# QWTforGithub/CDSegNet

Hardware: AMD Instinct MI355X
Metric: points/sec/node (ScanNet ~120k-pt scenes, 1-step) (higher is better)
Workload: dtype f16

## Files before the change

### cdsegnet_amd/_lib.py

```python
import ctypes
import os
import threading
from ctypes import POINTER, Structure, c_char_p, c_float, c_int, c_int32, c_int64, c_long, c_size_t, c_uint64, c_void_p

HERE = os.path.dirname(os.path.abspath(__file__))
LIB_PATH = os.path.join(HERE, "libcdseg_hip.so")
LIB_PATH_F16 = os.path.join(HERE, "libcdseg_hip_f16.so")

F32, BF16 = 0, 1
ACT_NONE, ACT_GELU, ACT_SWISH = 0, 1, 2
ORDER_IDS = {"z": 0, "z-trans": 1, "hilbert": 2, "hilbert-trans": 3}
ERRORS = {-1: "CDSEG_ERR_ARG", -2: "CDSEG_ERR_LAUNCH", -3: "CDSEG_ERR_WORKSPACE", -4: "CDSEG_ERR_UNSUPPORTED"}


class CdsegError(RuntimeError):
    pass


class DuplicateVoxelsError(CdsegError):

    def __init__(self, msg, count):
        super().__init__(msg)
        self.count = int(count)

# ... 143 lines not shown
    "cdseg_attn_tail_rr": (c_int, [c_void_p, c_int, c_void_p, c_void_p, c_void_p, c_void_p, c_float, c_void_p, c_void_p,
                                   c_void_p, c_int, c_void_p, c_int, c_long, c_int, c_void_p]),
    "cdseg_cpe_head_rr2": (c_int, [c_void_p, c_int, c_void_p, c_void_p, c_void_p, c_void_p, c_void_p, c_int, c_void_p, c_int,
                                   c_void_p, c_void_p, c_void_p, c_float, c_void_p, c_void_p, c_int, c_long, c_int, c_int, c_void_p]),
    "cdseg_attn_tail_rr2": (c_int, [c_void_p, c_int, c_void_p, c_void_p, c_void_p, c_void_p, c_float, c_void_p, c_void_p,
                                    c_void_p, c_int, c_void_p, c_int, c_void_p, c_int, c_long, c_int, c_void_p, c_size_t, c_void_p]),
    "cdseg_block_scratch_bytes": (c_size_t, [POINTER(BlockDesc), c_long]),
    "cdseg_block_forward": (c_int, [POINTER(BlockDesc), POINTER(BlockIO), c_void_p]),
    "cdseg_layernorm": (c_int, [c_void_p, c_int, c_int, c_void_p, c_void_p, c_float, c_void_p, c_int, c_void_p,
                                c_void_p, c_int, c_int, c_void_p, c_int, c_int, c_long, c_int, c_void_p]),
    "cdseg_attention": (c_int, [c_void_p, c_void_p, c_void_p, c_int, c_int, c_int, c_void_p, c_void_p, c_void_p,
                                c_void_p, c_int, c_int, c_int, c_float, c_void_p, c_int, c_int, c_void_p]),
    "cdseg_attention_ex": (c_int, [c_void_p, c_void_p, c_void_p, c_int, c_int, c_int, c_void_p, c_void_p, c_void_p,
                                   c_void_p, c_int, c_int, c_int, c_float, c_void_p, c_int, c_int, c_int, c_void_p]),
    "cdseg_attention_schedule": (c_long, [c_int, c_int, c_int, c_int, c_void_p, c_long]),
    "cdseg_attention_bwd_ws_bytes": (c_size_t, [c_long, c_int]),
    "cdseg_attention_bwd": (c_int, [c_void_p, c_void_p, c_void_p, c_int, c_int, c_int, c_void_p, c_void_p, c_void_p, c_void_p,
                                    c_int, c_int, c_long, c_int, c_float, c_void_p, c_int, c_void_p, c_void_p, c_void_p,
                                    c_int, c_int, c_int, c_int, c_void_p, c_size_t, c_void_p]),
    "cdseg_layernorm_bwd": (c_int, [c_void_p, c_int, c_void_p, c_float, c_void_p, c_int, c_void_p, c_int, c_int, c_void_p,
                                    c_void_p, c_long, c_int, c_void_p]),
    "cdseg_gelu_bwd": (c_int, [c_void_p, c_void_p, c_void_p, c_long, c_void_p]),
    "cdseg_conv_wgrad": (c_int, [c_void_p, c_int, c_void_p, c_int, c_void_p, c_int, c_long, c_int, c_int, c_void_p, c_void_p,
                                 c_void_p]),
    "cdseg_linear_wgrad": (c_int, [c_void_p, c_int, c_void_p, c_void_p, c_int, c_long, c_int, c_int, c_void_p, c_int, c_void_p,
                                   c_void_p]),
    "cdseg_prof_enable": (c_int, [c_int]),
    "cdseg_prof_summary": (c_int, [POINTER(ctypes.c_double), POINTER(c_long)]),
    "cdseg_prof_summary_class": (c_int, [c_int, POINTER(ctypes.c_double), POINTER(c_long)]),
    "cdseg_segment_max": (c_int, [c_void_p, c_int, c_int, c_void_p, c_long, c_int, c_void_p, c_void_p, c_int,
# ... 74 lines not shown
```

### cdsegnet_amd/csrc/gemm.hip

```cpp
#include <cstdlib>

#include <atomic>

#include "common.h"
#include "prof.h"

#ifndef CDSEG_CONV_SQ128_MIN_M
#define CDSEG_CONV_SQ128_MIN_M 8000
#endif
#ifndef CDSEG_CONV_SQ128_MAX_M
#define CDSEG_CONV_SQ128_MAX_M 32768
#endif

namespace {

struct GemmP {
  const void* A;
  const void* W;
  const float* bias;
  const float* scale;
  const float* shift;
  const float* res;
  const float* add_src;
  const int32_t* add_idx;
// ... 1 lines not shown
  const int32_t* out_idx;
  void* out;
  void* out2;
  long M;
  int N, K, kvol;
  int lda, ldo, ldo2, ldres, ldadd;
  int out_dtype, out2_dtype;
  int act, out2_pre_add;
  int vec_ok;
  float* ws;
  int splits;
  int kshift;
  long nbr_sm, nbr_so;
  int gm, gn;
  int xmode;
  int fix;
  const float* colbias;
  const float* ln_pre_g;
  const float* ln_pre_b;
  const float* ln_post_g;
  const float* ln_post_b;
  void* ln_out;
  int ldln, ln_out_dtype;
  float ln_eps;
  int alt;
#ifdef CDSEG_EXPERIMENTS
  int dbg;
#endif
};

// ... 252 lines not shown
  const long groups = g.M * (long)(g.N >> 2);
  const long t = (long)blockIdx.x * blockDim.x + threadIdx.x;
  if (t >= groups) return;
  const long m = t / (g.N >> 2);
  const int n = (int)(t - m * (g.N >> 2)) << 2;
  const long stride = g.M * (long)g.N;
  const float* p = g.ws + m * g.N + n;
  float4 v = *reinterpret_cast<const float4*>(p);
  for (int s = 1; s < g.splits; ++s) {
    const float4 u = *reinterpret_cast<const float4*>(p + s * stride);
    v.x += u.x; v.y += u.y; v.z += u.z; v.w += u.w;
  }
  epilogue4(g, m, n, v);
}

__global__ __launch_bounds__(256) void row_finish_kernel(GemmP g) {
  const int lane = threadIdx.x & 63;
  const long m = (long)blockIdx.x * 4 + (threadIdx.x >> 6);
  if (m >= g.M) return;
  const int groups = g.N >> 2;
  const long sstride = g.M * (long)g.N;
  float4 v[2];
#pragma unroll
  for (int i = 0; i < 2; ++i) {
    v[i] = make_float4(0.f, 0.f, 0.f, 0.f);
    if (lane + 64 * i < groups) {
      const float* p = g.ws + m * g.N + 4 * (lane + 64 * i);
      v[i] = *reinterpret_cast<const float4*>(p);
      for (int s2 = 1; s2 < g.splits; ++s2) {
        const float4 u = *reinterpret_cast<const float4*>(p + s2 * sstride);
// ... 8 lines not shown
__device__ unsigned long long g_gemm_t[8 * 16384];
extern "C" int cdseg_debug_gemm_timing(unsigned long long* host_dst, size_t count) {
  return hipMemcpyFromSymbol(host_dst, HIP_SYMBOL(g_gemm_t), count * sizeof(unsigned long long)) == hipSuccess ? 0 : -2;
}
__device__ unsigned long long g_gemm_kt[4096 * 16 * 8];
extern "C" int cdseg_debug_gemm_ktiming(unsigned long long* host_dst, size_t count) {
  return hipMemcpyFromSymbol(host_dst, HIP_SYMBOL(g_gemm_kt), count * sizeof(unsigned long long)) == hipSuccess ? 0 : -2;
}
#define KT_STAMP(x) const unsigned long long x = __builtin_readcyclecounter()
#else
#define KT_STAMP(x)
#endif

template <int BN, int BM, bool SQ = false, int AI = 2, int AJ = BN / 32>
__device__ __forceinline__ void tile_epilogue(const GemmP& g, f32x4_t (&acc)[AI][AJ], char* smem, int tid, int lane,
                                              int wm, int wn, long m0, int n0, int zs) {
  constexpr int NT = SQ ? 512 : 4 * BM;
  constexpr int TN = BN / 32;
  constexpr int CLD = BN + 4;
  const int fr = lane & 15, fg = lane >> 4;
  float* Cs = reinterpret_cast<float*>(smem);
  const bool plain = !g.fix && plain_bf16_out(g);
  Cols8 cols;
  if (plain) cols = load_cols8(g, n0 + 8 * (tid % (BN / 8)));
  auto lds_barrier = [] {
    asm volatile("s_waitcnt lgkmcnt(0)" ::: "memory");
    __builtin_amdgcn_s_barrier();
  };
#pragma unroll 1
  for (int hh = 0; hh < BM / 64; ++hh) {
#ifdef CDSEG_GEMM_TIMING
    if (tid == 0 && blockIdx.x < 16384) g_gemm_t[(size_t)blockIdx.x * 8 + 4 + 2 * hh] = __builtin_readcyclecounter();
#endif
    if (hh) lds_barrier();
    int zcol = 0;
    if constexpr (BM > 64) asm volatile("v_mov_b32 %0, 0" : "=v"(zcol));
    if constexpr (SQ) {
// ... 9 lines not shown
      const int rbase = (wm & 1) * 32;
#pragma unroll
      for (int i = 0; i < 2; ++i)
#pragma unroll
        for (int j = 0; j < TN; ++j)
#pragma unroll
          for (int r = 0; r < 4; ++r)
            Cs[(rbase + i * 16 + fg * 4 + r) * CLD + wn * (BN / 2) + j * 16 + fr] = acc[i][j][r];
    }
    lds_barrier();
#ifdef CDSEG_GEMM_TIMING
    if (tid == 0 && blockIdx.x < 16384) g_gemm_t[(size_t)blockIdx.x * 8 + 5 + 2 * hh] = __builtin_readcyclecounter();
#endif
    const long mb = m0 + 64 * hh;
    constexpr int GPR = BN / 4;
    if (g.fix) {
      for (int item = tid; item < 64 * GPR; item += NT) {
        const int row = item / GPR, cg = item % GPR;
        const long m = mb + row;
        const int n = n0 + 4 * cg;
        if (m >= g.M || n >= g.N) continue;
        *reinterpret_cast<float4*>(g.ws + ((long)zs * g.M + m) * g.N + n) =
            *reinterpret_cast<const float4*>(Cs + row * CLD + 4 * cg);
      }
    } else if (BM == 64 && (g.ln_pre_g || g.ln_post_g)) {
      constexpr int MAXG = BN / 16;
      const int row = (tid >> 2) & 63, part = tid & 3;
      const long m = mb + row;
      const int ng = g.N >> 2;
      float4 v[MAXG];
#pragma unroll
      for (int i = 0; i < MAXG; ++i)
        v[i] = (part + 4 * i < ng) ? *reinterpret_cast<const float4*>(Cs + row * CLD + 4 * (part + 4 * i))
                                   : make_float4(0.f, 0.f, 0.f, 0.f);
      finish_row<MAXG>(g, m, m < g.M, part, 4, ng, 0, v);
    } else if (plain) {
      static_assert(NT % (GPR / 2) == 0, "a lane's columns must not change between items");
// ... 254 lines not shown
              for (int j = 0; j < TN; ++j)
                acc[i][j] = __builtin_amdgcn_mfma_f32_16x16x4f32(a[i][h][ss], b[j][h][ss], acc[i][j], 0, 0, 0);
      }
    }
    __syncthreads();
    if (kc + 1 < kc1) store_tiles();
    __syncthreads();
  }

  if constexpr (kIsX3<CT>) {
#pragma unroll
    for (int i = 0; i < 2; ++i)
#pragma unroll
      for (int j = 0; j < TN; ++j) acc[i][j] += accx[i][j] * (1.0f / 2048.f);
  }
  tile_epilogue<BN, BM>(g, acc, smem, tid, lane, wm, wn, m0, n0, zs);
}

__device__ uint4 g_zero_page[8];

template <int BM, bool GATHER = true, int BN = 128, int NST = 2, bool SQ = false>
struct DmaCfg {
  static constexpr int WAVES = SQ ? 8 : BM / 16, NT = WAVES * 64, BK = 64;
  static constexpr int A_BYTES = BM * 128, W_BYTES = BN * 128;
  static constexpr int A_PW = (BM / 8) / WAVES, W_PW = (BN / 8) / WAVES;
  static constexpr int STAGES = NST * (A_BYTES + W_BYTES);
  static constexpr int ITAB = GATHER ? BM * 27 * 4 : 0;
  static constexpr int LDS = STAGES + ITAB + 1024;
};

template <int BM, bool GATHER, int BN = 128, int NST = 2, bool SQ = false>
// ... 5 lines not shown
  constexpr int TN = BN / 32;
  constexpr int AI = SQ ? 4 : 2, AJ = TN;
  static_assert(!SQ || (BM == 256 && NST == 2 && GATHER), "SQ: 256-row tiles of 8 waves, two stages, sparse convs");
  extern __shared__ __attribute__((aligned(16))) char smem[];
  char* tail = smem + D::STAGES + D::ITAB;
  int* live = reinterpret_cast<int*>(tail);
  int* glive = reinterpret_cast<int*>(tail + 256);
  unsigned long long* smask = reinterpret_cast<unsigned long long*>(tail + 640);
  int* itab = reinterpret_cast<int*>(smem + D::STAGES);

  const int tid = threadIdx.x;
  const int lane = tid & 63;
  const int wave = __builtin_amdgcn_readfirstlane(tid >> 6);
  const int wm = wave >> 1, wn = wave & 1;
  int mt, sl;
  {
    const int bid = blockIdx.x, slices = g.gn * g.splits;
    if (g.xmode == 1) {
      const int j = bid >> 3;
      mt = j % g.gm;
      sl = (bid & 7) + 8 * (j / g.gm);
      if (sl >= slices) return;
    } else if (g.xmode == 2) {
      const int j = bid >> 3, chunk = (g.gm + 7) >> 3;
      mt = (bid & 7) * chunk + j / slices;
      sl = j % slices;
      if (j / slices >= chunk || mt >= g.gm) return;
    } else {
      mt = bid % g.gm;
      sl = bid / g.gm;
    }
  }
  const int nt = sl % g.gn, zs = sl / g.gn;
// ... 37 lines not shown
    __syncthreads();
    nlive = __builtin_amdgcn_readfirstlane(live[0]);
#pragma unroll
    for (int i = 0; i < PASSES; ++i) {
      const int o = og + OPT * i;
      if (o < g.kvol) {
        const int sl2 = slotmap[o];
        if (sl2 >= 0) itab[r * 27 + sl2] = idx[i];
      }
    }
    __syncthreads();
  }
  const int KV = nlive * g.K;
  const int nkc = KV / D::BK;
  const int kshift = g.kshift;
  const int kc0 = (int)(((long)nkc * zs) / g.splits);
  const int kc1 = (int)(((long)nkc * (zs + 1)) / g.splits);

  const int lrow = lane >> 3, slot = lane & 7;
  const bf16_t* a_src[D::A_PW];
  int a_row[D::A_PW];
  int a_chunk[D::A_PW];
  const bf16_t* w_src[D::W_PW];
  int w_chunk[D::W_PW];
#pragma unroll
  for (int i = 0; i < D::A_PW; ++i) {
    const int r = (wave * D::A_PW + i) * 8 + lrow;
    a_row[i] = r;
    a_chunk[i] = slot ^ ((r >> 1) & 7);
    long m = m0 + r;
    if (m >= g.M) m = g.M - 1;
    a_src[i] = (const bf16_t*)g.A + m * g.lda + a_chunk[i] * 8;
// ... 217 lines not shown
  }
#ifdef CDSEG_GEMM_TIMING
  if (lane == 0 && blockIdx.x < 4096 && wave < 16) {
    unsigned long long* d = g_gemm_kt + ((size_t)blockIdx.x * 16 + wave) * 8;
    d[0] = kt_wait; d[1] = kt_bar; d[2] = kt_issue; d[3] = kt_mma; d[4] = (unsigned long long)(kc1 - kc0); d[5] = kt_pro;
    d[6] = (unsigned long long)nlive; d[7] = 1;
  }
#endif
  __syncthreads();
#ifdef CDSEG_EXPERIMENTS
  if (g.dbg & 4) { if (acc[0][0][0] == 12345.678f) ((float*)g.out)[0] = acc[1][1][1]; return; }
#endif
#ifdef CDSEG_GEMM_TIMING
  const unsigned long long tc1 = __builtin_readcyclecounter();
#endif
  tile_epilogue<BN, BM, SQ, AI, AJ>(g, acc, smem, tid, lane, wm, wn, m0, n0, zs);
#ifdef CDSEG_GEMM_TIMING
  if (tid == 0 && blockIdx.x < 16384) {
    unsigned long long* d = g_gemm_t + (size_t)blockIdx.x * 8;
    d[0] = rt0; d[1] = __builtin_amdgcn_s_memrealtime(); d[2] = tc1 - tc0;
    const unsigned long long tend = __builtin_readcyclecounter();
    d[3] = tend - tc1;
    const unsigned long long a0 = d[4], a1 = d[5], b0 = d[6], b1 = d[7];
    d[4] = a1 - a0; d[5] = b0 - a1; d[6] = b1 - b0; d[7] = tend - b1;
  }
#endif
}

thread_local bool tl_leave_partials = false;
thread_local int tl_partial_splits = 1;

template <typename CT, int BN, int NCH, int BM>
constexpr int gemm_smem_bytes() {
  constexpr int ab = (BM + BN) * NCH * 16, c = 64 * (BN + 4) * 4;
  return (ab > c ? ab : c) + 1024;
}


template <typename CT, int NCH, bool GATHER>
int launch_bn(GemmP p, size_t ws_bytes, hipStream_t s) {
  constexpr int BK = NCH * (16 / (int)sizeof(CT));
  static const int split_target = cdseg_knob("CDSEG_GEMM_SPLIT_TARGET", 320);
  static const int split_max = cdseg_knob("CDSEG_GEMM_SPLIT_MAX", 16);
  static const int xmode_env = cdseg_knob("CDSEG_GEMM_XMODE", -1);
  const bool ln = p.ln_pre_g || p.ln_post_g;
// ... 71 lines not shown
  else if (ln && gn > 1) p.fix = 2;
  if (p.fix) {
    if (!can_fix || (size_t)splits * p.M * p.N * sizeof(float) > ws_bytes) return CDSEG_ERR_WORKSPACE;
    if (p.fix == 2 && p.N > 512) return CDSEG_ERR_UNSUPPORTED;
  }
  p.splits = splits;
  p.gm = gm;
  p.gn = gn;
  const int slices = gn * splits;
  const long wbytes = (long)p.N * p.kvol * p.K * (long)sizeof(CT);
  p.xmode = 0;
  if (sq) p.xmode = gm >= 64 ? 2 : 0;
  else if (slices >= 8 && wbytes >= (1 << 20) && gm > 1) p.xmode = 1;
  else if (GATHER && gm >= 64) p.xmode = 2;
  if (xmode_env >= 0) p.xmode = (xmode_env == 1 && slices < 8) ? 0 : xmode_env;
  unsigned nblk;
  if (p.xmode == 1) nblk = 8u * (unsigned)((slices + 7) / 8) * (unsigned)gm;
  else if (p.xmode == 2) nblk = 8u * (unsigned)((gm + 7) / 8) * (unsigned)slices;
  else nblk = (unsigned)gm * (unsigned)slices;
  const dim3 grid(nblk);
  bool launched = false;
  if constexpr (NCH == 16 && sizeof(CT) == 2) {
    static const int dma_on = cdseg_knob("CDSEG_GEMM_DMA", 1);
    static const int dma_bm = cdseg_knob("CDSEG_GEMM_DMA_BM", 0);
    const bool fused_ln_here = ln && gn == 1 && splits == 1;
    if constexpr (GATHER) {
      if (sq && dma_on && sq_bn == 128) {
        launched = true;
        using Q = DmaCfg<256, true, 128, 2, true>;
        static std::atomic<bool> aq128{false};
        if (!aq128) {
          if (hipFuncSetAttribute((const void*)gemm_dma_kernel<256, true, 128, 2, true>, hipFuncAttributeMaxDynamicSharedMemorySize,
// ... 117 lines not shown
            attr_x3 = true;
          }
          hipLaunchKernelGGL((gemm_kernel<CT, 128, NCH, false, 128>), grid, dim3(512), smem, s, p);
        } else {
          hipLaunchKernelGGL((gemm_kernel<CT, 128, NCH, false, 128>), grid, dim3(512), 0, s, p);
        }
      }
    }
  }
  if (!launched) {
    if (bn == 32) hipLaunchKernelGGL((gemm_kernel<CT, 32, NCH, GATHER>), grid, dim3(256), 0, s, p);
    else if (bn == 64) hipLaunchKernelGGL((gemm_kernel<CT, 64, NCH, GATHER>), grid, dim3(256), 0, s, p);
    else hipLaunchKernelGGL((gemm_kernel<CT, 128, NCH, GATHER>), grid, dim3(256), 0, s, p);
  }
  if (hipGetLastError() != hipSuccess) return CDSEG_ERR_LAUNCH;
  if (p.fix == 2) {
    hipLaunchKernelGGL(row_finish_kernel, dim3((unsigned)((p.M + 3) / 4)), dim3(256), 0, s, p);
    if (hipGetLastError() != hipSuccess) return CDSEG_ERR_LAUNCH;
  } else if (p.fix == 1) {
    if (tl_leave_partials && p.vec_ok && p.bias && !p.scale && p.act == CDSEG_ACT_NONE && !p.res && !p.add_src && !p.out2 &&
        !p.out_idx && !p.colbias) {
      tl_partial_splits = p.splits;
      return CDSEG_OK;
    }
    const long groups = p.M * (long)(p.N >> 2);
    hipLaunchKernelGGL(splitk_epilogue_kernel, dim3((unsigned)((groups + 255) / 256)), dim3(256), 0, s, p);
    if (hipGetLastError() != hipSuccess) return CDSEG_ERR_LAUNCH;
  }
  return CDSEG_OK;
}
// ... 39 lines not shown
  p.colbias = a->colbias; p.ln_pre_g = a->ln_pre_g; p.ln_pre_b = a->ln_pre_b; p.ln_post_g = a->ln_post_g;
  p.ln_post_b = a->ln_post_b; p.ln_out = a->ln_out; p.ldln = a->ldln; p.ln_out_dtype = a->ln_out_dtype;
  p.ln_eps = a->ln_eps;
  if (p.ln_pre_g || p.ln_post_g) {
    if (a->N > 512 || !p.vec_ok || a->out_idx || (p.ln_pre_g && !p.ln_pre_b) || (p.ln_post_g && (!p.ln_post_b || !a->ln_out)) ||
        (a->ln_out && (a->ldln % 4)))
      return CDSEG_ERR_UNSUPPORTED;
  }
  if (p.colbias && !al16(p.colbias)) p.vec_ok = 0;
  p.ws = (a->ws && ((((uintptr_t)a->ws) & 15) == 0)) ? (float*)a->ws : nullptr;
  p.splits = 1;
  p.fix = 0;
  p.alt = cdseg_knob("CDSEG_GEMM_ALT", 0);
  p.gm = p.gn = 1;
  p.xmode = 0;
  p.kshift = -1;
  if ((a->K & (a->K - 1)) == 0) {
    int sh = 0;
    while ((1 << sh) < a->K) ++sh;
    p.kshift = sh;
  }
  const size_t wsb = p.ws ? a->ws_bytes : 0;
  hipStream_t s = (hipStream_t)stream;
  CdsegProfToken tok;
  const bool prof = a->nbr && a->kvol == 27 && cdseg_prof_begin(CDSEG_PROF_CONV_DEEP, s, &tok);
  int rc = CDSEG_ERR_ARG;
  if (a->compute_dtype == CDSEG_BF16) rc = a->nbr ? launch<bf16_t, true>(p, wsb, s) : launch<bf16_t, false>(p, wsb, s);
  else if (a->compute_dtype == CDSEG_F32) rc = a->nbr ? launch<float, true>(p, wsb, s) : launch<float, false>(p, wsb, s);
  else if (a->compute_dtype == CDSEG_F32X3) rc = a->nbr ? launch<F32X3, true>(p, wsb, s) : launch<F32X3, false>(p, wsb, s);
  if (prof) cdseg_prof_end(tok, s);
  return rc;
}

int gemm_leave_partials(const cdseg_gemm_args* a, int* splits, void* stream) {
  tl_leave_partials = true;
  tl_partial_splits = 1;
  const int rc = cdseg_gemm(a, stream);
  tl_leave_partials = false;
  *splits = tl_partial_splits;
  return rc;
}
```

### cdsegnet_amd/csrc/runtime.hip

```cpp
#include <cstdlib>
#include <cstring>

#include "common.h"
#include "deep.h"

namespace {

inline size_t align_up(size_t v, size_t a) { return (v + a - 1) / a * a; }

struct Carver {
  char* base;
  size_t off, cap;
  void* take(size_t bytes) {
    off = align_up(off, 256);
    void* p = base ? base + off : nullptr;
    off += bytes;
    return p;
  }
};

constexpr int FUSE_LN_MAX_C = 512;
constexpr size_t SPLITK_WS_CAP = (size_t)64 << 20;

inline size_t esz(int dtype) { return dtype == CDSEG_BF16 ? 2 : 4; }
// ... 11 lines not shown
  Layout L;
  L.y = c.take(n * C * e);
  L.h = c.take(n * C * e);
  L.qkv = c.take(n * 3 * C * e);
  L.o = c.take(n * C * e);
  L.u = c.take(n * (size_t)d->hidden * e);
  L.y2 = d->channels > FUSE_LN_MAX_C ? c.take(n * C * 4) : nullptr;
  const long tiles = ((n + 63) / 64) * (((long)C + 127) / 128);
  L.ws_bytes = tiles < 256 ? (size_t)32 * n * (size_t)(3 * C > (size_t)d->hidden ? 3 * C : d->hidden) * 4
                           : (C > 128 ? (size_t)n * C * 4 : 0);
  if (C >= 256 && ((n + 127) / 128) * (((long)C + 255) / 256) < 256) {
    const size_t want = (size_t)8 * n * C * 4;
    if (want > L.ws_bytes) L.ws_bytes = want;
  }
  if (L.ws_bytes > SPLITK_WS_CAP) L.ws_bytes = SPLITK_WS_CAP;
  L.ws = L.ws_bytes ? c.take(L.ws_bytes) : nullptr;
  L.xs = (d->dtype == CDSEG_BF16 && C >= 128 && d->head_img && d->tail_img) ? c.take(n * C * 4) : nullptr;
  L.total = align_up(c.off, 256);
  return L;
}

cdseg_gemm_args base_args(const cdseg_block_desc* d, const Layout& L, long n) {
  cdseg_gemm_args a;
  std::memset(&a, 0, sizeof(a));
  a.M = n;
  a.kvol = 1;
  a.a_dtype = storage_dtype(d->dtype);
  a.compute_dtype = d->dtype;
  a.ws = L.ws;
  a.ws_bytes = L.ws_bytes;
// ... 192 lines not shown
```

### cdsegnet_amd/ops.py

```python
import ctypes
import os
import threading

import torch

from . import _lib
from ._lib import ACT_GELU, ACT_NONE, ACT_SWISH, BF16, F32, GemmArgs, check

__all__ = ["ACT_NONE", "ACT_GELU", "ACT_SWISH", "F32", "BF16"]

LP_DTYPES = {"bf16": torch.bfloat16, "f16": torch.float16}


class _Dtypes:

    def __getitem__(self, dtype):
        if dtype == torch.float32:
            return F32
        if dtype == LP_DTYPES[_lib.active()]:
            return BF16
        raise _lib.CdsegError(f"{dtype} tensors do not belong to the active build of the library ({_lib.active()})")


_DT = _Dtypes()
# ... 441 lines not shown
        patch = (ctypes.c_int * k)(*[int(it[3]) for it in chunk])
        npad = (ctypes.c_long * k)(*[int(it[4]) for it in chunk])
        check(lib.cdseg_pad_plan_batch(k, orders, offs, offs_pad, patch, npad, int(nb), _ptr(gidx), _ptr(widx), _stream()),
              "pad_plan_batch")
        sizes = [int(it[4]) for it in chunk]
        res.extend(zip(gidx.split(sizes), widx.split(sizes)))
    return res


F32X3 = 2


def set_f32x3(on):
    prev, _TLS.f32x3 = _TLS.f32x3, bool(on)
    return prev


def gemm(A, W, out, *, bias=None, scale=None, shift=None, act=ACT_NONE, res=None, add_src=None, add_idx=None,
         nbr=None, out_idx=None, out2=None, out2_pre_add=False, M=None, kvol=1, colbias=None, ln_pre=None,
         nbr_kmajor=False,
         ln_post=None, ln_out=None, ln_eps=1e-5, cache=True):
    if not A.is_cuda:
        _need_gpu(A, W, out)
    x3 = _TLS.f32x3 and W.dtype == torch.float32
    key = (W.data_ptr(), _dp(bias), _dp(scale), _dp(shift), int(kvol), int(act), x3)
    cache_d = _TLS.gemm_cache
    ent = cache_d.get(key) if cache else None
    if ent is None:
        for t in (bias, scale, shift):
            if t is not None and t.dtype != torch.float32:
# ... 27 lines not shown
    a.a_dtype = _DT[A.dtype]
    a.out_dtype = _DT[out.dtype]
    a.out2_dtype = _DT[out2.dtype] if out2 is not None else 0
    a.out2_pre_add = 1 if out2_pre_add else 0
    a.colbias = _dp(colbias)
    if ln_pre is not None:
        a.ln_pre_g, a.ln_pre_b = ln_pre[0].data_ptr(), ln_pre[1].data_ptr()
    else:
        a.ln_pre_g = a.ln_pre_b = None
    if ln_post is not None:
        a.ln_post_g, a.ln_post_b = ln_post[0].data_ptr(), ln_post[1].data_ptr()
        a.ln_out, a.ldln, a.ln_out_dtype = ln_out.data_ptr(), ln_out.stride(0), _DT[ln_out.dtype]
    else:
        a.ln_post_g = a.ln_post_b = a.ln_out = None
    a.ln_eps = float(ln_eps)
    if ((m + 63) >> 6) * ((a.N + 127) >> 7) < 256:
        ws = workspace(min(32 * m * a.N * 4, 64 << 20), out.device)
        a.ws, a.ws_bytes = ws.data_ptr(), ws.numel()
    elif nbr is not None and a.N >= 256 and ((m + 127) >> 7) * ((a.N + 255) >> 8) < 256:
        ws = workspace(min(8 * m * a.N * 4, 64 << 20), out.device)
        a.ws, a.ws_bytes = ws.data_ptr(), ws.numel()
    elif a.N > 128 and (ln_pre is not None or ln_post is not None):
        ws = workspace(m * a.N * 4, out.device)
        a.ws, a.ws_bytes = ws.data_ptr(), ws.numel()
    else:
        a.ws, a.ws_bytes = None, 0
    tok = TIMER.begin("conv" if nbr is not None else "gemm") if TIMER is not None else None
    check(_lib.load().cdseg_gemm(ent[1], _stream()), "gemm")
    if tok is not None:
        TIMER.end(tok, 2.0 * a.M * a.N * a.K * a.kvol)
    return out


FUSED_MLP_CHANNELS = (32, 64, 128)

# ... 534 lines not shown
```

### include/cdseg.h

```cpp
#ifndef CDSEG_H
#define CDSEG_H

#include <stddef.h>
#include <stdint.h>

#ifdef __cplusplus
extern "C" {
#endif

#define CDSEG_OK 0
#define CDSEG_ERR_ARG (-1)
#define CDSEG_ERR_LAUNCH (-2)
#define CDSEG_ERR_WORKSPACE (-3)
#define CDSEG_ERR_UNSUPPORTED (-4)

#define CDSEG_F32 0
#define CDSEG_BF16 1
#define CDSEG_F32X3 2

#define CDSEG_ORDER_Z 0
#define CDSEG_ORDER_Z_TRANS 1
#define CDSEG_ORDER_HILBERT 2
#define CDSEG_ORDER_HILBERT_TRANS 3

// ... 98 lines not shown
int cdseg_layernorm(const void* x, int x_dtype, int ldx, const float* gamma, const float* beta, float eps,
                    const float* res, int ldres, const float* colbias, void* out, int out_dtype, int ldo,
                    void* out2, int out2_dtype, int ldo2, long m, int c, void* stream);

int cdseg_attention(const void* q, const void* k, const void* v, int ldq, int ldk, int ldv, const int32_t* q_gidx,
                    const int32_t* kv_gidx, const int32_t* widx, const int32_t* patch_start, int num_patches,
                    int num_heads, int max_len, float scale, void* out, int ldo, int dtype, void* stream);
#define CDSEG_ATTN_Q_PRESCALED 1
#define CDSEG_ATTN_V_BF16 2
int cdseg_attention_ex(const void* q, const void* k, const void* v, int ldq, int ldk, int ldv, const int32_t* q_gidx,
                       const int32_t* kv_gidx, const int32_t* widx, const int32_t* patch_start, int num_patches,
                       int num_heads, int max_len, float scale, void* out, int ldo, int dtype, int flags, void* stream);

long cdseg_attention_schedule(int num_patches, int num_heads, int max_len, int dtype, int32_t* table, long capacity);

int cdseg_prof_enable(int on);
int cdseg_prof_summary(double* total_ms, long* launches);
#define CDSEG_PROF_ATTENTION 0
#define CDSEG_PROF_CONV 1
#define CDSEG_PROF_CONV_DEEP 2
int cdseg_prof_summary_class(int cls, double* total_ms, long* launches);

int cdseg_segment_max(const void* y, int y_dtype, int ldy, const int32_t* seg_start, long m, int c,
                      const float* scale, const float* shift, int act, float* out, int ldo, void* out2,
                      int out2_dtype, int ldo2, void* stream);
size_t cdseg_pool_fused_img_bytes(int cin, int cout);
int cdseg_pool_fused_pack(const void* w, int cin, int cout, void* wimg, void* stream);
int cdseg_pool_fused(const void* x, int ldx, const void* wimg, const float* bias, const int32_t* seg_start, long m,
                     const float* scale, const float* shift, int act, float* out, int ldo, void* out2, int ldo2,
                     int cin, int cout, void* stream);
// ... 213 lines not shown
```

Baseline: 79.83 million.

## Add cost-model split plan for sparse conv GEMM with per-tile mixed split-K

Adds a host-side planner that picks, per XCD, how many output tiles run whole and how many are split across K into S or S+1 pieces, replacing uniform split-K for 256x256 gathered bf16 convolutions. The goal is to balance the tail of the wave across compute slots and cut partial-sum traffic compared with splitting every tile. Partial tiles are written to a compact workspace and reduced by a new epilogue kernel. This adds planning cost (cached), extra workspace sizing in Python and the runtime, and depends on hand-tuned cost constants.

```diff
diff --git a/cdsegnet_amd/_lib.py b/cdsegnet_amd/_lib.py
--- a/cdsegnet_amd/_lib.py
+++ b/cdsegnet_amd/_lib.py
@@ -181,6 +181,8 @@
     "cdseg_attention_ex": (c_int, [c_void_p, c_void_p, c_void_p, c_int, c_int, c_int, c_void_p, c_void_p, c_void_p,
                                    c_void_p, c_int, c_int, c_int, c_float, c_void_p, c_int, c_int, c_int, c_void_p]),
     "cdseg_attention_schedule": (c_long, [c_int, c_int, c_int, c_int, c_void_p, c_long]),
+    "cdseg_conv_split_plan_ws_bytes": (c_size_t, [c_long, c_int, c_int]),
+    "cdseg_debug_conv_split_plan": (c_long, [c_long, c_int, c_int, c_size_t, c_void_p, POINTER(c_size_t), c_void_p, c_long]),
     "cdseg_attention_bwd_ws_bytes": (c_size_t, [c_long, c_int]),
     "cdseg_attention_bwd": (c_int, [c_void_p, c_void_p, c_void_p, c_int, c_int, c_int, c_void_p, c_void_p, c_void_p, c_void_p,
                                     c_int, c_int, c_long, c_int, c_float, c_void_p, c_int, c_void_p, c_void_p, c_void_p,
diff --git a/cdsegnet_amd/csrc/gemm.hip b/cdsegnet_amd/csrc/gemm.hip
--- a/cdsegnet_amd/csrc/gemm.hip
+++ b/cdsegnet_amd/csrc/gemm.hip
@@ -1,6 +1,9 @@
 #include <cstdlib>
 
+#include <algorithm>
 #include <atomic>
+#include <mutex>
+#include <vector>
 
 #include "common.h"
 #include "prof.h"
@@ -39,6 +42,7 @@
   long nbr_sm, nbr_so;
   int gm, gn;
   int xmode;
+  int pw, pnb, ps;
   int fix;
   const float* colbias;
   const float* ln_pre_g;
@@ -321,6 +325,72 @@
   epilogue4(g, m, n, v);
 }
 
+struct PlanXcd {
+  int row0, w, nb, nc;
+  int chi;
+};
+__host__ __device__ __forceinline__ PlanXcd plan_xcd(int gm, int gn, int pw, int pnb, int x) {
+  const int base = gm >> 3, rem = gm & 7;
+  const int T = (base + (x < rem ? 1 : 0)) * gn, thi = (base + (rem ? 1 : 0)) * gn;
+  const int whi = pw < thi ? pw : thi;
+  PlanXcd o;
+  o.row0 = x * base + (x < rem ? x : rem);
+  o.w = pw < T ? pw : T;
+  o.nb = pnb < T - o.w ? pnb : T - o.w;
+  o.nc = T - o.w - o.nb;
+  o.chi = thi - whi - (pnb < thi - whi ? pnb : thi - whi);
+  return o;
+}
+struct PlanPiece {
+  int mt, nt, a, S;
+  int wt;
+};
+__host__ __device__ __forceinline__ bool plan_decode(int gm, int gn, int pw, int pnb, int ps, int bid, PlanPiece& o) {
+  const int x = bid & 7, j = bid >> 3;
+  const PlanXcd c = plan_xcd(gm, gn, pw, pnb, x);
+  int t;
+  if (j < c.w) {
+    t = j; o.a = 0; o.S = 1; o.wt = -1;
+  } else if (j < c.w + c.nb * ps) {
+    const int jj = j - c.w, a = jj / c.nb, k = jj - a * c.nb;
+    t = c.w + k; o.a = a; o.S = ps; o.wt = (a * 8 + x) * pnb + k;
+  } else {
+    const int jj = j - c.w - c.nb * ps;
+    if (jj >= c.nc * (ps + 1)) return false;
+    const int a = jj / c.nc, k = jj - a * c.nc;
+    t = c.w + c.nb + k; o.a = a; o.S = ps + 1; o.wt = 8 * pnb * ps + (a * 8 + x) * c.chi + k;
+  }
+  o.mt = c.row0 + t / gn;
+  o.nt = t - (t / gn) * gn;
+  return true;
+}
+
+template <int BM, int BN>
+__global__ __launch_bounds__(256) void plan_epilogue_kernel(GemmP g) {
+  const PlanXcd c0 = plan_xcd(g.gm, g.gn, g.pw, g.pnb, 0);
+  const int per = g.pnb + c0.chi;
+  const int x = blockIdx.y / per, k = blockIdx.y - x * per;
+  const PlanXcd c = plan_xcd(g.gm, g.gn, g.pw, g.pnb, x);
+  const bool late = k >= g.pnb;
+  const int kk = late ? k - g.pnb : k;
+  if (kk >= (late ? c.nc : c.nb)) return;
+  const int t = c.w + (late ? c.nb : 0) + kk, S = g.ps + (late ? 1 : 0);
+  const long slot0 = late ? (long)8 * g.pnb * g.ps + x * c.chi + kk : (long)x * g.pnb + kk;
+  const long sstride = (long)8 * (late ? c.chi : g.pnb) * (BM * BN);
+  const int item = blockIdx.x * 256 + threadIdx.x;
+  const int row = item / (BN / 4), cg = item - row * (BN / 4);
+  const long m = (long)(c.row0 + t / g.gn) * BM + row;
+  const int n = (t % g.gn) * BN + 4 * cg;
+  if (m >= g.M || n >= g.N) return;
+  const float* p = g.ws + slot0 * (BM * BN) + row * BN + 4 * cg;
+  float4 v = *reinterpret_cast<const float4*>(p);
+  for (int s = 1; s < S; ++s) {
+    const float4 u = *reinterpret_cast<const float4*>(p + s * sstride);
+    v.x += u.x; v.y += u.y; v.z += u.z; v.w += u.w;
+  }
+  epilogue4(g, m, n, v);
+}
+
 __global__ __launch_bounds__(256) void row_finish_kernel(GemmP g) {
   const int lane = threadIdx.x & 63;
   const long m = (long)blockIdx.x * 4 + (threadIdx.x >> 6);
@@ -359,13 +429,13 @@
 
 template <int BN, int BM, bool SQ = false, int AI = 2, int AJ = BN / 32>
 __device__ __forceinline__ void tile_epilogue(const GemmP& g, f32x4_t (&acc)[AI][AJ], char* smem, int tid, int lane,
-                                              int wm, int wn, long m0, int n0, int zs) {
+                                              int wm, int wn, long m0, int n0, int fix, float* wsp, long wld) {
   constexpr int NT = SQ ? 512 : 4 * BM;
   constexpr int TN = BN / 32;
   constexpr int CLD = BN + 4;
   const int fr = lane & 15, fg = lane >> 4;
   float* Cs = reinterpret_cast<float*>(smem);
-  const bool plain = !g.fix && plain_bf16_out(g);
+  const bool plain = !fix && plain_bf16_out(g);
   Cols8 cols;
   if (plain) cols = load_cols8(g, n0 + 8 * (tid % (BN / 8)));
   auto lds_barrier = [] {
@@ -405,13 +475,13 @@
 #endif
     const long mb = m0 + 64 * hh;
     constexpr int GPR = BN / 4;
-    if (g.fix) {
+    if (fix) {
       for (int item = tid; item < 64 * GPR; item += NT) {
         const int row = item / GPR, cg = item % GPR;
         const long m = mb + row;
         const int n = n0 + 4 * cg;
         if (m >= g.M || n >= g.N) continue;
-        *reinterpret_cast<float4*>(g.ws + ((long)zs * g.M + m) * g.N + n) =
+        *reinterpret_cast<float4*>(wsp + (long)(64 * hh + row) * wld + 4 * cg) =
             *reinterpret_cast<const float4*>(Cs + row * CLD + 4 * cg);
       }
     } else if (BM == 64 && (g.ln_pre_g || g.ln_post_g)) {
@@ -696,7 +766,7 @@
 #pragma unroll
       for (int j = 0; j < TN; ++j) acc[i][j] += accx[i][j] * (1.0f / 2048.f);
   }
-  tile_epilogue<BN, BM>(g, acc, smem, tid, lane, wm, wn, m0, n0, zs);
+  tile_epilogue<BN, BM>(g, acc, smem, tid, lane, wm, wn, m0, n0, g.fix, g.ws + ((long)zs * g.M + m0) * g.N + n0, g.N);
 }
 
 __device__ uint4 g_zero_page[8];
@@ -732,9 +802,14 @@
   const int wave = __builtin_amdgcn_readfirstlane(tid >> 6);
   const int wm = wave >> 1, wn = wave & 1;
   int mt, sl;
+  int pS = 0, pz = 0, pwt = -1;
   {
     const int bid = blockIdx.x, slices = g.gn * g.splits;
-    if (g.xmode == 1) {
+    if (SQ && g.xmode == 3) {
+      PlanPiece pp;
+      if (!plan_decode(g.gm, g.gn, g.pw, g.pnb, g.ps, bid, pp)) return;
+      mt = pp.mt; sl = pp.nt; pS = pp.S; pz = pp.a; pwt = pp.wt;
+    } else if (g.xmode == 1) {
       const int j = bid >> 3;
       mt = j % g.gm;
       sl = (bid & 7) + 8 * (j / g.gm);
@@ -802,8 +877,13 @@
   const int KV = nlive * g.K;
   const int nkc = KV / D::BK;
   const int kshift = g.kshift;
-  const int kc0 = (int)(((long)nkc * zs) / g.splits);
-  const int kc1 = (int)(((long)nkc * (zs + 1)) / g.splits);
+  int kc0 = (int)(((long)nkc * zs) / g.splits);
+  int kc1 = (int)(((long)nkc * (zs + 1)) / g.splits);
+  if (SQ && pS) {
+    const int q = nkc / pS, r = nkc - q * pS;
+    kc0 = pz * q + (pz < r ? pz : r);
+    kc1 = kc0 + q + (pz < r ? 1 : 0);
+  }
 
   const int lrow = lane >> 3, slot = lane & 7;
   const bf16_t* a_src[D::A_PW];
@@ -1051,7 +1131,12 @@
 #ifdef CDSEG_GEMM_TIMING
   const unsigned long long tc1 = __builtin_readcyclecounter();
 #endif
-  tile_epilogue<BN, BM, SQ, AI, AJ>(g, acc, smem, tid, lane, wm, wn, m0, n0, zs);
+  {
+    const bool planned = SQ && pS;
+    const int fix = planned ? (pwt >= 0 ? 1 : 0) : g.fix;
+    float* wsp = planned ? g.ws + (long)pwt * (BM * BN) : g.ws + ((long)zs * g.M + m0) * g.N + n0;
+    tile_epilogue<BN, BM, SQ, AI, AJ>(g, acc, smem, tid, lane, wm, wn, m0, n0, fix, wsp, planned ? (long)BN : (long)g.N);
+  }
 #ifdef CDSEG_GEMM_TIMING
   if (tid == 0 && blockIdx.x < 16384) {
     unsigned long long* d = g_gemm_t + (size_t)blockIdx.x * 8;
@@ -1066,6 +1151,136 @@
 
 thread_local bool tl_leave_partials = false;
 thread_local int tl_partial_splits = 1;
+
+constexpr double PLAN_STEP_US = 1.65;
+constexpr double PLAN_PARTIAL_US = 0.11;
+constexpr double PLAN_PASS_US = 2.0;
+constexpr int PLAN_PIECE_STEPS = 3;
+constexpr int PLAN_SLOTS = 32;
+constexpr int PLAN_MAX_S = 7;
+constexpr double PLAN_MIN_GAIN = 0.03;
+constexpr size_t PLAN_TILE_BYTES = (size_t)256 * 256 * 4;
+
+struct SplitPlan {
+  int uniform;
+  int pw, pnb, ps;
+  int nblk;
+  int makespan;
+  int partials;
+  long ws_tiles;
+  double cost_us;
+};
+
+int plan_makespan(int T, int pw, int pnb, int ps, int nkc) {
+  const int w = pw < T ? pw : T, nb = pnb < T - w ? pnb : T - w, nc = T - w - nb;
+  int slot[PLAN_SLOTS] = {0};
+  int end = 0;
+  auto put = [&](int len) {
+    int b = 0;
+    for (int i = 1; i < PLAN_SLOTS; ++i)
+      if (slot[i] < slot[b]) b = i;
+    slot[b] += len + PLAN_PIECE_STEPS;
+    if (slot[b] > end) end = slot[b];
+  };
+  for (int i = 0; i < w; ++i) put(nkc);
+  for (int cls = 0; cls < 2; ++cls) {
+    const int S = ps + cls, cnt = cls ? nc : nb;
+    if (!cnt) continue;
+    const int q = nkc / S, r = nkc - q * S;
+    for (int a = 0; a < S; ++a)
+      for (int k = 0; k < cnt; ++k) put(q + (a < r ? 1 : 0));
+  }
+  return end;
+}
+
+SplitPlan conv_split_plan(int gm, int gn, int nkc, size_t ws_bytes, int usplits, bool leave) {
+  struct Key { int gm, gn, nkc, us, leave; size_t cap; };
+  struct Ent { Key k; SplitPlan p; };
+  static std::mutex mu;
+  static std::vector<Ent> cache;
+  const Key key{gm, gn, nkc, usplits, leave ? 1 : 0, ws_bytes / PLAN_TILE_BYTES};
+  {
+    std::lock_guard<std::mutex> lk(mu);
+    for (const Ent& e : cache)
+      if (e.k.gm == key.gm && e.k.gn == key.gn && e.k.nkc == key.nkc && e.k.us == key.us && e.k.leave == key.leave &&
+          e.k.cap == key.cap)
+        return e.p;
+  }
+  const int base = gm >> 3, rem = gm & 7;
+  const int thi = (base + (rem ? 1 : 0)) * gn, tlo = base * gn;
+  SplitPlan best;
+  best.uniform = 1; best.pw = best.pnb = best.ps = 0; best.nblk = 0; best.partials = 0; best.ws_tiles = 0;
+  {
+    const long per = gm >= 64 ? (long)((gm + 7) / 8) * gn * usplits : ((long)gm * gn * usplits + 7) / 8;
+    const int len = (nkc + usplits - 1) / usplits + PLAN_PIECE_STEPS;
+    best.makespan = (int)((per + PLAN_SLOTS - 1) / PLAN_SLOTS) * len;
+    best.cost_us = best.makespan * PLAN_STEP_US;
+    if (usplits > 1) best.cost_us += (double)gm * gn * usplits * PLAN_PARTIAL_US + (leave ? 0.0 : PLAN_PASS_US);
+  }
+  const double need = best.cost_us * (1.0 - PLAN_MIN_GAIN);
+  SplitPlan plan = best;
+  plan.cost_us = 1e30;
+  struct Cand { double floor_us, fixed; int pw, pnb, ps, parts; long tiles; };
+  std::vector<Cand> cands;
+  for (int pw = thi > 48 ? thi - 48 : 0; pw <= thi; ++pw) {
+    const int R = thi - pw;
+    for (int ps = 2; ps <= PLAN_MAX_S; ++ps) {
+      if (nkc / (ps + 1) < 8) break;
+      if (R == 0 && ps > 2) break;
+      for (int pnb = (R && ps > 2) ? 1 : 0; pnb <= R; ++pnb) {
+        const PlanXcd c = plan_xcd(gm, gn, pw, pnb, 0);
+        const long tiles = (long)8 * pnb * ps + (long)8 * c.chi * (ps + 1);
+        if ((size_t)tiles > ws_bytes / PLAN_TILE_BYTES) continue;
+        int parts = 0;
+        for (int x = 0; x < 8; ++x) {
+          const PlanXcd cx = plan_xcd(gm, gn, pw, pnb, x);
+          parts += cx.nb * ps + cx.nc * (ps + 1);
+        }
+        const long work = (long)c.w * (nkc + PLAN_PIECE_STEPS) + (long)c.nb * (nkc + ps * PLAN_PIECE_STEPS) +
+                          (long)c.nc * (nkc + (ps + 1) * PLAN_PIECE_STEPS);
+        const double fixed = parts * PLAN_PARTIAL_US + (parts ? PLAN_PASS_US : 0.0);
+        const double floor_us = (double)((work + PLAN_SLOTS - 1) / PLAN_SLOTS) * PLAN_STEP_US + fixed;
+        if (floor_us < need) cands.push_back(Cand{floor_us, fixed, pw, pnb, ps, parts, tiles});
+      }
+    }
+  }
+  std::sort(cands.begin(), cands.end(), [](const Cand& a, const Cand& b) {
+    if (a.floor_us != b.floor_us) return a.floor_us < b.floor_us;
+    if (a.parts != b.parts) return a.parts < b.parts;
+    return a.pw != b.pw ? a.pw < b.pw : (a.ps != b.ps ? a.ps < b.ps : a.pnb < b.pnb);
+  });
+  for (const Cand& cd : cands) {
+    if (cd.floor_us >= plan.cost_us) break;
+    int ms = plan_makespan(thi, cd.pw, cd.pnb, cd.ps, nkc);
+    if (tlo != thi && tlo > 0) {
+      const int m2 = plan_makespan(tlo, cd.pw, cd.pnb, cd.ps, nkc);
+      if (m2 > ms) ms = m2;
+    }
+    const double cost = ms * PLAN_STEP_US + cd.fixed;
+    if (cost < plan.cost_us) {
+      const PlanXcd c = plan_xcd(gm, gn, cd.pw, cd.pnb, 0);
+      plan.uniform = 0; plan.pw = cd.pw; plan.pnb = cd.pnb; plan.ps = cd.ps; plan.makespan = ms; plan.partials = cd.parts;
+      plan.ws_tiles = cd.tiles; plan.cost_us = cost;
+      plan.nblk = 8 * (c.w + c.nb * cd.ps + c.nc * (cd.ps + 1));
+    }
+  }
+  if (plan.cost_us < need) best = plan;
+  std::lock_guard<std::mutex> lk(mu);
+  if (cache.size() > 256) cache.clear();
+  cache.push_back(Ent{key, best});
+  return best;
+}
+
+int sq_uniform_splits(long M, int N, int K, int gm, int gn, size_t ws_bytes) {
+  const long nkc128 = ((long)27 * K + 127) / 128, blocks = (long)gm * gn;
+  if (blocks >= 256 || nkc128 < 4) return 1;
+  int smax = (int)(nkc128 / 2);
+  if (smax > 16) smax = 16;
+  while (smax > 1 && (size_t)smax * M * N * sizeof(float) > ws_bytes) --smax;
+  int splits = (int)(256 / blocks);
+  if (splits > smax) splits = smax;
+  return splits < 1 ? 1 : splits;
+}
 
 template <typename CT, int BN, int NCH, int BM>
 constexpr int gemm_smem_bytes() {
@@ -1167,8 +1382,37 @@
   else if (slices >= 8 && wbytes >= (1 << 20) && gm > 1) p.xmode = 1;
   else if (GATHER && gm >= 64) p.xmode = 2;
   if (xmode_env >= 0) p.xmode = (xmode_env == 1 && slices < 8) ? 0 : xmode_env;
+  SplitPlan plan;
+  plan.uniform = 1;
+  if constexpr (GATHER && NCH == 16 && sizeof(CT) == 2) {
+    static const int plan_on = cdseg_knob("CDSEG_CONV_SPLIT_PLAN", 1);
+    if (plan_on && sq && sq_bn == 256 && can_fix && xmode_env < 0 && p.fix != 2) {
+      const bool leave = tl_leave_partials && p.bias && !p.scale && p.act == CDSEG_ACT_NONE && !p.res && !p.add_src && !p.out2 &&
+                         !p.colbias;
+      plan = conv_split_plan(gm, gn, (int)((long)p.kvol * p.K / 64), ws_bytes, splits, leave);
+#ifdef CDSEG_EXPERIMENTS
+      if (const int fps = cdseg_knob("CDSEG_PLAN_PS", 0); fps > 0) {
+        const int fpw = cdseg_knob("CDSEG_PLAN_PW", 0), fpnb = cdseg_knob("CDSEG_PLAN_PNB", 0);
+        const PlanXcd c = plan_xcd(gm, gn, fpw, fpnb, 0);
+        const long tiles = (long)8 * fpnb * fps + (long)8 * c.chi * (fps + 1);
+        if ((size_t)tiles <= ws_bytes / PLAN_TILE_BYTES) {
+          plan.uniform = 0; plan.pw = fpw; plan.pnb = fpnb; plan.ps = fps; plan.ws_tiles = tiles;
+          plan.partials = c.nb + c.nc;
+          plan.nblk = 8 * (c.w + c.nb * fps + c.nc * (fps + 1));
+        }
+      }
+#endif
+      if (!plan.uniform) {
+        p.splits = 1;
+        p.fix = 0;
+        p.xmode = 3;
+        p.pw = plan.pw; p.pnb = plan.pnb; p.ps = plan.ps;
+      }
+    }
+  }
   unsigned nblk;
-  if (p.xmode == 1) nblk = 8u * (unsigned)((slices + 7) / 8) * (unsigned)gm;
+  if (p.xmode == 3) nblk = (unsigned)plan.nblk;
+  else if (p.xmode == 1) nblk = 8u * (unsigned)((slices + 7) / 8) * (unsigned)gm;
   else if (p.xmode == 2) nblk = 8u * (unsigned)((gm + 7) / 8) * (unsigned)slices;
   else nblk = (unsigned)gm * (unsigned)slices;
   const dim3 grid(nblk);
@@ -1316,6 +1560,14 @@
     else hipLaunchKernelGGL((gemm_kernel<CT, 128, NCH, GATHER>), grid, dim3(256), 0, s, p);
   }
   if (hipGetLastError() != hipSuccess) return CDSEG_ERR_LAUNCH;
+  if (p.xmode == 3) {
+    if (plan.partials) {
+      const unsigned per = (unsigned)(p.pnb + plan_xcd(gm, gn, p.pw, p.pnb, 0).chi);
+      hipLaunchKernelGGL((plan_epilogue_kernel<256, 256>), dim3(256 * 256 / 1024, 8u * per), dim3(256), 0, s, p);
+      if (hipGetLastError() != hipSuccess) return CDSEG_ERR_LAUNCH;
+    }
+    return CDSEG_OK;
+  }
   if (p.fix == 2) {
     hipLaunchKernelGGL(row_finish_kernel, dim3((unsigned)((p.M + 3) / 4)), dim3(256), 0, s, p);
     if (hipGetLastError() != hipSuccess) return CDSEG_ERR_LAUNCH;
@@ -1385,6 +1637,7 @@
   p.alt = cdseg_knob("CDSEG_GEMM_ALT", 0);
   p.gm = p.gn = 1;
   p.xmode = 0;
+  p.pw = p.pnb = p.ps = 0;
   p.kshift = -1;
   if ((a->K & (a->K - 1)) == 0) {
     int sh = 0;
@@ -1411,3 +1664,37 @@
   *splits = tl_partial_splits;
   return rc;
 }
+
+extern "C" size_t cdseg_conv_split_plan_ws_bytes(long M, int N, int K) {
+  if (M < 5000 || N < 256 || (N % 256) || K <= 0 || (K & (K - 1)) || K < 64) return 0;
+  const int gm = (int)((M + 255) / 256), gn = N / 256;
+  const size_t big = ~(size_t)0 >> 1;
+  const SplitPlan pl = conv_split_plan(gm, gn, 27 * K / 64, big, sq_uniform_splits(M, N, K, gm, gn, big), false);
+  return pl.uniform ? 0 : (size_t)pl.ws_tiles * PLAN_TILE_BYTES;
+}
+
+extern "C" long cdseg_debug_conv_split_plan(long M, int N, int K, size_t ws_bytes, int32_t* hdr, size_t* ws_need, int32_t* pieces,
+                                            long capacity) {
+  if (!hdr || !ws_need || M < 5000 || N < 256 || (N % 256) || K <= 0 || (K & (K - 1)) || K < 64) return CDSEG_ERR_ARG;
+  const int gm = (int)((M + 255) / 256), gn = N / 256, nkc = 27 * K / 64;
+  const int us = sq_uniform_splits(M, N, K, gm, gn, ws_bytes);
+  const SplitPlan pl = conv_split_plan(gm, gn, nkc, ws_bytes, us, false);
+  const int h[12] = {pl.uniform, us, gm, gn, nkc, pl.pw, pl.pnb, pl.ps, pl.nblk, pl.makespan, pl.partials, 0};
+  for (int i = 0; i < 12; ++i) hdr[i] = h[i];
+  *ws_need = pl.uniform ? (us > 1 ? (size_t)us * M * N * sizeof(float) : 0) : (size_t)pl.ws_tiles * PLAN_TILE_BYTES;
+  if (pl.uniform) return 0;
+  for (long b = 0; b < pl.nblk && b < capacity && pieces; ++b) {
+    int32_t* o = pieces + 6 * b;
+    PlanPiece pp;
+    if (!plan_decode(gm, gn, pl.pw, pl.pnb, pl.ps, (int)b, pp)) {
+      for (int i = 0; i < 6; ++i) o[i] = -1;
+      continue;
+    }
+    const int q = nkc / pp.S, r = nkc - q * pp.S;
+    o[0] = (int)(b & 7); o[1] = pp.mt; o[2] = pp.nt;
+    o[3] = pp.a * q + (pp.a < r ? pp.a : r);
+    o[4] = o[3] + q + (pp.a < r ? 1 : 0);
+    o[5] = pp.wt;
+  }
+  return pl.nblk;
+}
diff --git a/cdsegnet_amd/csrc/runtime.hip b/cdsegnet_amd/csrc/runtime.hip
--- a/cdsegnet_amd/csrc/runtime.hip
+++ b/cdsegnet_amd/csrc/runtime.hip
@@ -49,6 +49,10 @@
     if (want > L.ws_bytes) L.ws_bytes = want;
   }
   if (L.ws_bytes > SPLITK_WS_CAP) L.ws_bytes = SPLITK_WS_CAP;
+  if (C >= 256 && d->dtype == CDSEG_BF16) {
+    const size_t want = cdseg_conv_split_plan_ws_bytes(n, (int)C, (int)C);
+    if (want > L.ws_bytes) L.ws_bytes = want;
+  }
   L.ws = L.ws_bytes ? c.take(L.ws_bytes) : nullptr;
   L.xs = (d->dtype == CDSEG_BF16 && C >= 128 && d->head_img && d->tail_img) ? c.take(n * C * 4) : nullptr;
   L.total = align_up(c.off, 256);
diff --git a/cdsegnet_amd/ops.py b/cdsegnet_amd/ops.py
--- a/cdsegnet_amd/ops.py
+++ b/cdsegnet_amd/ops.py
@@ -479,6 +479,19 @@
 def set_f32x3(on):
     prev, _TLS.f32x3 = _TLS.f32x3, bool(on)
     return prev
+
+
+_PLAN_WS = {}
+
+
+def _conv_plan_ws(m, n, k):
+    key = (m, n, k, _lib.active())
+    v = _PLAN_WS.get(key)
+    if v is None:
+        if len(_PLAN_WS) > 4096:
+            _PLAN_WS.clear()
+        v = _PLAN_WS[key] = int(_lib.load().cdseg_conv_split_plan_ws_bytes(m, n, k))
+    return v
 
 
 def gemm(A, W, out, *, bias=None, scale=None, shift=None, act=ACT_NONE, res=None, add_src=None, add_idx=None,
@@ -536,11 +549,15 @@
     else:
         a.ln_post_g = a.ln_post_b = a.ln_out = None
     a.ln_eps = float(ln_eps)
+    plan_ws = _conv_plan_ws(m, a.N, a.K) if nbr is not None and a.kvol == 27 and a.N >= 256 and a.N == a.K and is_lp(W.dtype) else 0
     if ((m + 63) >> 6) * ((a.N + 127) >> 7) < 256:
-        ws = workspace(min(32 * m * a.N * 4, 64 << 20), out.device)
+        ws = workspace(max(min(32 * m * a.N * 4, 64 << 20), plan_ws), out.device)
         a.ws, a.ws_bytes = ws.data_ptr(), ws.numel()
     elif nbr is not None and a.N >= 256 and ((m + 127) >> 7) * ((a.N + 255) >> 8) < 256:
-        ws = workspace(min(8 * m * a.N * 4, 64 << 20), out.device)
+        ws = workspace(max(min(8 * m * a.N * 4, 64 << 20), plan_ws), out.device)
+        a.ws, a.ws_bytes = ws.data_ptr(), ws.numel()
+    elif plan_ws:
+        ws = workspace(plan_ws, out.device)
         a.ws, a.ws_bytes = ws.data_ptr(), ws.numel()
     elif a.N > 128 and (ln_pre is not None or ln_post is not None):
         ws = workspace(m * a.N * 4, out.device)
diff --git a/include/cdseg.h b/include/cdseg.h
--- a/include/cdseg.h
+++ b/include/cdseg.h
@@ -136,6 +136,10 @@
 
 long cdseg_attention_schedule(int num_patches, int num_heads, int max_len, int dtype, int32_t* table, long capacity);
 
+size_t cdseg_conv_split_plan_ws_bytes(long M, int N, int K);
+long cdseg_debug_conv_split_plan(long M, int N, int K, size_t ws_bytes, int32_t* hdr, size_t* ws_need, int32_t* pieces,
+                                 long capacity);
+
 int cdseg_prof_enable(int on);
 int cdseg_prof_summary(double* total_ms, long* launches);
 #define CDSEG_PROF_ATTENTION 0
```

Result: no change. 79.18 million (-0.8%).
